# akshatvasisht/janus

Hardware: AMD Instinct MI355X
Metric: xRT (audio-s/wall-s) per GPU, 30s clips batch=64; p50 encode+decode latency (higher is better)
Workload: dtype fp16

## Files before the change

### include/janus_kernels.h

```cpp
#ifndef JANUS_KERNELS_H_
#define JANUS_KERNELS_H_

#include <stddef.h>
#include <stdint.h>
#include "janus.h"

#ifdef __cplusplus
extern "C" {
#endif

enum { JANUS_EPI_F16 = 0, JANUS_EPI_GELU_F16 = 1, JANUS_EPI_RESID_F32 = 2, JANUS_EPI_F32 = 3 };
enum { JANUS_ACT_NONE = 0, JANUS_ACT_SILU = 1, JANUS_ACT_GELU = 2, JANUS_ACT_TANH = 3 };

int janus_gemm_f16(int epi, const uint16_t* A, int64_t lda, const uint16_t* W, int64_t ldw,
                   const float* bias, void* C, int64_t ldc, const float* R, int64_t ldr, int M,
                   int N, int K, void* stream);

int janus_gemm_nt128_f16(int epi, const uint16_t* A, int64_t lda, const uint16_t* W, int64_t ldw,
                         const float* bias, void* C, int64_t ldc, const float* R, int64_t ldr, int M,
                         int N, int K, void* stream);

int janus_gemm_lt_f16(int epi, const uint16_t* A, int64_t lda, const uint16_t* W, int64_t ldw,
                      const float* bias, void* C, int64_t ldc, const float* R, int64_t ldr, int M,
                      int N, int K, void* stream);
// ... 38 lines not shown

int janus_cross_attention_f16(const uint16_t* qk, const uint16_t* enc, int batch, int Te, int D,
                              int H, int nsplit, float* part_c, float* part_ml, uint16_t* out,
                              void* stream);

int janus_decode_attention_f16(const uint16_t* q, int64_t q_bs, const uint16_t* k,
                               const uint16_t* v, int64_t kv_bs, int64_t kv_rs, int Tkv,
                               uint16_t* out, int64_t o_bs, int batch, int H, float scale,
                               float* part_o, float* part_ml, void* stream);

int janus_np_voiced_mean_f32(const float* values, const int64_t* offsets, int batch,
                             float* mean_out, int32_t* count_out, void* stream);

int janus_sample_gumbel_f32(const uint32_t* seeds, int batch, int pos, int V, float* out,
                            void* stream);

int janus_beam_partial_blocks(int V, int K, int max_blocks);
int janus_beam_logits_topk_f16(const uint16_t* A, const uint16_t* W, int K, int V, int batch,
                               int eot, int suppress_blank, int blank, int ts_begin,
                               int no_timestamps, int max_initial_ts, const uint8_t* smask,
                               const int32_t* row_rules, int max_blocks, void* parts, void* tops,
                               int n2k, float* all_v, int32_t* all_i, float* ts_v, int32_t* ts_i,
                               void* stream);
int janus_beam_step(const void* parts, const void* tops, int nblk, int eot, int suppress_blank,
                    int blank, int ts_begin, int no_timestamps, int max_initial_ts,
                    int32_t* row_rules, int32_t* tokens, int ld, int pos, int32_t* done,
                    float* sum_lp, int32_t* n_tok, const int32_t* plen, int beam_size,
                    int n_windows, int32_t* nlive, int32_t* nfin, int32_t* wdone, int32_t* moved,
                    int32_t* parent, int32_t* fin_tok, float* fin_s, int32_t* fin_n, void* stream);
int janus_beam_reorder_f16(uint16_t* kc, uint16_t* vc, int layers, int n_windows, int beam_size,
                           int n_ctx, int d, int pos, const int32_t* parent, const int32_t* moved,
                           void* stream);

int janus_decode_plan_describe(const janus_whisper_config* cfg, const janus_decode_options* opt,
                               const janus_decode_rows* rows, int batch, int cus, int resident,
                               int multi_lane, float temperature, const float* temperatures,
                               int beam_size, const int32_t* stand, int n_stand, int stand_maxlen,
                               char* text, int text_cap, int64_t* key, int key_cap, int32_t* n_key);

int janus_align_dtw_f32(const float* x, int N, int F, uint8_t* trace, int32_t* text_indices,
                        int32_t* time_indices, int32_t* path_len, void* stream);
int janus_align_reduce_f32(const float* probs, int heads, int n, int F, int sot_len, float* A,
                           void* stream);
int janus_align_token_prob_f16(const float* x, const float* gamma, const float* beta,
                               const uint16_t* W, int rows, int d, int V, const int32_t* target,
                               float* prob, void* stream);

int janus_lang_head_f16(const float* x, const float* gamma, const float* beta, const uint16_t* emb,
                        int d, int lang_begin, int n_lang, int rows, float* probs, int32_t* best,
                        void* stream);

#ifdef __cplusplus
}
#endif
#endif
```

### janus_amd/_native.py

```python
import ctypes

import numpy as np
import os

import torch

LIB_PATH = os.path.join(os.path.dirname(os.path.abspath(__file__)), "libjanus_hip.so")
if os.environ.get("JANUS_LIB"):
    LIB_PATH = os.path.join(os.path.dirname(os.path.abspath(__file__)), os.path.basename(os.environ["JANUS_LIB"]))


class JanusNativeError(RuntimeError):
    """A libjanus_hip.so entry point returned a non-zero status."""


class janus_value(ctypes.Structure):
    _fields_ = [("type", ctypes.c_int32), ("i", ctypes.c_int64), ("f", ctypes.c_double),
                ("s", ctypes.c_char_p), ("len", ctypes.c_size_t)]


class janus_packet(ctypes.Structure):
    _fields_ = [("text", ctypes.c_char_p), ("text_len", ctypes.c_size_t),
                ("mode", ctypes.c_int64), ("n_prosody", ctypes.c_int32),
                ("prosody_keys", ctypes.POINTER(janus_value)),
# ... 60 lines not shown
    "janus_vocoder_set_tensor": [_P, ctypes.c_char_p, _P, _I64],
    "janus_vocoder_frontend": [_P, _P, _P, _P, _I32, _I32, _P, _P],
    "janus_vocoder_frontend_ex": [_P, _P, _P, _P, _P, _I32, _I32, _P, _P],
    "janus_vocoder_speaker": [_P, _P, _P, _I32, _P, _P],
    "janus_vocoder_forward": [_P, _P, _I32, _I32, _P, _P, _P],
    "janus_vocoder_forward_ex": [_P, _P, _I32, _I32, _P, _P, _P, _P],
    "janus_vocoder_set_timing": [_P, _I32],
    "janus_vocoder_conv_stats": [_P, _P, _P, _P, _I32],
    "janus_vocoder_family_stats": [_P, _I32, _P, _P, _P, _P, _P, _P, _I32],
    "janus_gemm_f16": [_I32, _P, _I64, _P, _I64, _P, _P, _I64, _P, _I64, _I32, _I32, _I32, _P],
    "janus_gemm_nt128_f16": [_I32, _P, _I64, _P, _I64, _P, _P, _I64, _P, _I64, _I32, _I32, _I32, _P],
    "janus_gemm_lt_f16": [_I32, _P, _I64, _P, _I64, _P, _P, _I64, _P, _I64, _I32, _I32, _I32, _P],
    "janus_layernorm_f16": [_P, _P, _P, _P, _I32, _I32, _F32, _P],
    "janus_wave_xor_f32": [_P, _P, _I32, _P],
    "janus_quant_rows_i8": [_P, _I64, _P, _I64, _P, _I32, _I32, _P],
    "janus_layernorm_quant_i8": [_P, _P, _P, _P, _P, _I32, _I32, _F32, _P],
    "janus_gemm_i8": [_I32, _P, _I64, _P, _I64, _P, _P, _P, _P, _I64, _P, _I64, _I32, _I32, _I32, _P],
    "janus_resid_ln_f16": [_P, _I64, _P, _I64, _P, _P, _P, _P, _F32, _P, _I32, _I32, _I32, _P],
    "janus_gemm_ln_f16": [_I32, _P, _I64, _P, _P, _F32, _P, _I64, _P, _P, _I64, _I32, _I32, _I32, _P],
    "janus_attention_f16": [_P, _P, _I32, _I32, _I32, _F32, _P],
    "janus_conv1d_packed_size": [_I32, _I32, _I32, _I32, _I32],
    "janus_conv1d_pack": [_P, _P, _I32, _I32, _I32, _I32, _I32, _P],
    "janus_conv1d_f16": [_P, _I32, _I32, _I32, _P, _P, _P, _I32, _I32, _I32, _I32, _I32, _I32,
                         _I32, _I32, _I32, _P, _I64, _F32, _I32, _P],
    "janus_resunit_packed_size": [_I32, _I32],
    "janus_resunit_pack": [_P, _P, _I32, _I32, _P],
    "janus_resunit_f16": [_P, _P, _P, _P, _P, _P, _I32, _I32, _I32, _I32, _I32, _F32, _I32, _P],
    "janus_cross_attention_f16": [_P, _P, _I32, _I32, _I32, _I32, _I32, _P, _P, _P, _P],
    "janus_decode_attention_f16": [_P, _I64, _P, _P, _I64, _I64, _I32, _P, _I64, _I32, _I32, _F32,
                                   _P, _P, _P],
    "janus_beam_partial_blocks": [_I32, _I32, _I32],
    "janus_beam_logits_topk_f16": [_P, _P, _I32, _I32, _I32, _I32, _I32, _I32, _I32, _I32, _I32, _P, _P,
                                   _I32, _P, _P, _I32, _P, _P, _P, _P, _P],
    "janus_beam_step": [_P, _P, _I32, _I32, _I32, _I32, _I32, _I32, _I32, _P, _P, _I32, _I32, _P, _P, _P,
                        _P, _I32, _I32, _P, _P, _P, _P, _P, _P, _P, _P, _P],
    "janus_beam_reorder_f16": [_P, _P, _I32, _I32, _I32, _I32, _I32, _I32, _P, _P, _P],
    "janus_align_dtw_f32": [_P, _I32, _I32, _P, _P, _P, _P, _P],
    "janus_align_reduce_f32": [_P, _I32, _I32, _I32, _I32, _P, _P],
    "janus_align_token_prob_f16": [_P, _P, _P, _P, _I32, _I32, _I32, _P, _P, _P],
    "janus_whisper_detect_language": [_P, _P, _I32, _I32, _I32, _I32, _P, _P, _P],
    "janus_lang_head_f16": [_P, _P, _P, _P, _I32, _I32, _I32, _I32, _P, _P, _P],
    "janus_decode_plan_describe": [_P, _P, _P, _I32, _I32, _I32, _I32, _F32, _P, _I32, _P, _I32, _I32,
                                   _P, _I32, _P, _I32, _P],
}
RESTYPES = {"janus_conv1d_packed_size": ctypes.c_int64}

_lib = None


def lib() -> ctypes.CDLL:
    global _lib
    if _lib is None:
        if not os.path.exists(LIB_PATH):
            raise ImportError(
                f"{LIB_PATH} is missing: build it with `python -c 'import __graft_entry__ as g; "
                "g.build()'` (hipcc --offload-arch=gfx950). janus_amd has no CPU fallback.")
        l = ctypes.CDLL(LIB_PATH)
        l.janus_last_error.restype = ctypes.c_char_p
        l.janus_last_error.argtypes = []
        for name, argtypes in SIGNATURES.items():
            if os.environ.get("JANUS_LIB") and not hasattr(l, name):
                continue
            fn = getattr(l, name)
            fn.argtypes = argtypes
            fn.restype = RESTYPES.get(name, ctypes.c_int)
        _lib = l
    return _lib


def check(rc: int) -> None:
    if rc != 0:
        raise JanusNativeError(lib().janus_last_error().decode("utf-8", "replace"))


def call(name: str, *args) -> None:
    check(getattr(lib(), name)(*args))


# ... 55 lines not shown
```

### janus_amd/csrc/decode.cpp

```cpp
#include <algorithm>
#include <condition_variable>
#include <cstring>
#include <thread>
#include <type_traits>
#include "decoder.h"
#include "dec_persist.h"
#include "decode_plan.h"
#include "whisper_internal.h"

namespace janus {

struct LaneLatch {
  std::mutex m;
  std::condition_variable cv;
  int left = 0;
  void arrive(bool wait) {
    std::unique_lock<std::mutex> lk(m);
    if (--left == 0) cv.notify_all();
    if (wait) cv.wait(lk, [&] { return left <= 0; });
  }
};
struct LaneArrival {
  LaneLatch* l;
  bool done = false;
// ... 407 lines not shown
    _Float16* ck = ckeys + (int64_t)l * Me * d;
    _Float16* cv = cvals + (int64_t)l * Me * d;
    if (fused_ln) {
      gemm_skinny_ln_launch(EPI_F16, lnargs(L.ln2g, L.ln2b, L.wq_c.as<_Float16>(), L.bq_c, q2, d, d,
                                            nullptr, nullptr, pos), s);
    } else {
      if (!ln_fuse && !lnp2 && !rln2) layernorm_launch(x, L.ln2g, L.ln2b, a, B, d, 1e-5f, s);
      gemm_launch(EPI_F16, with_ln(dgargs(a, d, L.wq_c.as<_Float16>(), d, L.bq_c, q2, d, B, d, d),
                                   L.ln2g, L.ln2b, lnp2), s);
    }
    decode_attention_split_launch(q2, d, ck, cv, (int64_t)Te * d, d, Te, o, d, B, H, scale, part_o,
                                  part_ml, s);
    if (rln3) resid_ln(o, L.wo_c, L.bo_c, L.ln3g, L.ln3b);
    else resid(o, d, L.wo_c, L.bo_c, L.ln3g, L.ln3b);
  }

  void mlp(int l, int pos) const {
    DecLayer& L = w->dec[l];
    if (fused_ln) {
      gemm_skinny_ln_launch(EPI_GELU_F16, lnargs(L.ln3g, L.ln3b, L.w1.as<_Float16>(), L.b1, f, 4 * d,
                                                 4 * d, nullptr, nullptr, pos), s);
    } else {
      if (!ln_fuse && !lnp3 && !rln3) layernorm_launch(x, L.ln3g, L.ln3b, a, B, d, 1e-5f, s);
      gemm_launch(EPI_GELU_F16, with_ln(dgargs(a, d, L.w1.as<_Float16>(), d, L.b1, f, 4 * d, B, 4 * d, d),
                                        L.ln3g, L.ln3b, lnp3), s);
    }
    resid(f, 4 * d, L.w2, L.b2, l + 1 < nl ? w->dec[l + 1].ln1g : fin_g,
          l + 1 < nl ? w->dec[l + 1].ln1b : fin_b);
  }

  void tail(int pos) const {
    const int nblk = P.nblk, nwin = P.nwin;
    if (!ln_fuse && !lnp_fin && !layerk) layernorm_launch(x, fin_g, fin_b, a, B, d, 1e-5f, s);
    logits_partial_launch(a, d, w->tok16.as<_Float16>(), d, V, B, R, smask,
                          rules, parts, s,
                          lnp_fin ? x : nullptr, d, fin_g, fin_b, P.lg_cap,
                          P.sampling ? seed : nullptr, pos,
                          P.row_temps ? itemp : nullptr,
                          P.beam_k ? btop : nullptr);
    if (P.beam_k) {
      beam_step_launch(parts, btop, nblk, R, rules,
                       tokens, maxlen, pos, done, sum_lp, n_tokens, prompt,
                       nsp, bst, nwin, s);
      if (pos + 1 < maxlen - 1)
        beam_reorder_launch(kcache, vcache, nl, nwin, P.beam_k, NC, d, pos,
                            bst.parent, bst.moved, s);
      return;
    }
    if (P.fuse_se && pos + 1 < maxlen - 1)
      select_embed_launch(parts, nblk, R, rules, tokens,
                          maxlen, pos, done, sum_lp, n_tokens, B, s, prompt,
                          nsp, w->tok16.as<_Float16>(), pos_emb, d, x,
                          fused_ln ? lnp : nullptr, w->dec[0].ln1g, w->dec[0].ln1b,
                          (ln_fuse || (embed_ln && !layerk)) ? a : nullptr, roff);
    else
      select_partials_launch(parts, nblk, R, rules, tokens,
                             maxlen, pos, done, sum_lp, n_tokens, B, s, prompt,
                             nsp, roff);
  }

  void forward(int pos) const {
    if (!(P.fuse_se && pos >= P.sample_begin && pos > 0))
      embed_launch(w->tok16.as<_Float16>(), pos_emb, tokens, maxlen, pos, d, x,
                   fused_ln ? lnp : nullptr, B, s, w->dec[0].ln1g, w->dec[0].ln1b,
                   (ln_fuse || (embed_ln && !layerk)) ? a : nullptr, roff);
    for (int l = 0; l < nl; ++l) {
      DecLayer& L = w->dec[l];
// ... 429 lines not shown
```

### janus_amd/csrc/decoder.h

```cpp
#pragma once
#include "common.h"
#include "decode_shapes.h"

namespace janus {

struct RowRules {
  int sample_begin;
  int suppress_all_ts;
  int suppress_text;
  int ts_floor;
  int last_stamp;
  int pad[3];
};

struct LogitPart {
  float m_all, s_all;
  float m_text;
  float m_ts, s_ts;
  float b_all_v; int b_all_i;
  float b_ts_v; int b_ts_i;
  float t_v;
  float m_raw, s_raw;
  float b_all_r, b_ts_r;
};
// ... 4 lines not shown
  float tv[kBeamTop]; int ti[kBeamTop];
};

__host__ __device__ inline uint32_t noise_mix(uint32_t h) {
  h ^= h >> 16; h *= 0x85ebca6bu; h ^= h >> 13; h *= 0xc2b2ae35u; h ^= h >> 16;
  return h;
}
__host__ __device__ inline uint32_t noise_base(uint32_t seed, int pos) {
  return noise_mix(seed ^ noise_mix((uint32_t)pos * 0x9e3779b9u + 0x7f4a7c15u));
}
__device__ inline float sample_gumbel(uint32_t base, int token) {
  const uint32_t h = noise_mix(base ^ ((uint32_t)token * 0x27d4eb2fu));
  const float u = (float)((h >> 8) | 1u) * 0x1p-24f;
  return -logf(-logf(u));
}

void cast_f16_f32_launch(const _Float16* in, float* out, int64_t n, hipStream_t s);
void cast_f32_f16_launch(const float* in, _Float16* out, int64_t n, hipStream_t s);
void embed_launch(const _Float16* tok_emb, const float* pos_emb, const int32_t* tokens,
                  int ld_tokens, int pos, int d, float* x, float2* part, int B, hipStream_t s,
                  const float* ln_g = nullptr, const float* ln_b = nullptr,
                  _Float16* ln_out = nullptr, const int32_t* roff = nullptr);
void kv_store_launch(const _Float16* qkv, int d, int pos, int n_ctx, _Float16* kc, _Float16* vc,
                     int B, hipStream_t s);
void init_tokens_launch(int32_t* tokens, int ld, const int32_t* prompt, int plen, int32_t* done,
                        float* sum_lp, int32_t* n_tok, int B, hipStream_t s);
void init_counters_launch(int32_t* done, float* sum_lp, int32_t* n_tok, float* nsp, int B,
                          hipStream_t s);
void select_launch(const float* logits, int V, const DecodeRules& R, const uint8_t* smask,
                   int32_t* tokens, int ld, int pos, int sample_begin_pos, int32_t* done,
                   float* sum_lp, int32_t* n_tok, int B, hipStream_t s);
void rules_init_launch(RowRules* rules, int B, hipStream_t s);
int logits_partial_blocks(int V, int K, int max_blocks = 256);
void logits_partial_launch(const _Float16* A, int lda, const _Float16* W, int K, int V, int B,
                           const DecodeRules& R, const uint8_t* smask, const RowRules* rules,
                           LogitPart* parts, hipStream_t s,
                           const float* lnx = nullptr, int ldx = 0, const float* ln_g = nullptr,
                           const float* ln_b = nullptr, int max_blocks = 256,
                           const uint32_t* seeds = nullptr, int pos = 0,
                           const float* row_inv_temp = nullptr, BeamTop* tops = nullptr);
void select_partials_launch(const LogitPart* parts, int nblk, const DecodeRules& R,
                            RowRules* rules, int32_t* tokens, int ld, int pos, int32_t* done,
                            float* sum_lp, int32_t* n_tok, int B, hipStream_t s,
                            const int32_t* plen = nullptr, float* nsp = nullptr,
                            const int32_t* roff = nullptr);
void select_embed_launch(const LogitPart* parts, int nblk, const DecodeRules& R, RowRules* rules,
                         int32_t* tokens, int ld, int pos, int32_t* done, float* sum_lp,
                         int32_t* n_tok, int B, hipStream_t s, const int32_t* plen, float* nsp,
                         const _Float16* tok_emb, const float* pos_emb, int d, float* x,
                         float2* part, const float* ln_g, const float* ln_b, _Float16* ln_out,
                         const int32_t* roff = nullptr);
void build_mask_launch(const int32_t* list, int n, uint8_t* mask, int V, hipStream_t s);
void sample_gumbel_launch(const uint32_t* seeds, int B, int pos, int V, float* out, hipStream_t s);

struct BeamState {
  int k;
  float length_penalty;
  int32_t* nlive;
  int32_t* nfin;
  int32_t* wdone;
  int32_t* moved;
  int32_t* parent;
  int32_t* fin_tok;
  float* fin_s;
  int32_t* fin_n;
};
void beam_init_launch(const BeamState& st, int W, hipStream_t s);
// ... 15 lines not shown
```

### janus_amd/csrc/decoder.hip

```cpp
#include <algorithm>
#include <cfloat>
#include <cstdlib>
#ifdef JANUS_DEBUG_ASSERT
#include <cassert>
#endif
#include "mfma.h"
#include "kernels.h"
#include "decoder.h"
#include "decoder_dev.h"

namespace janus {

__global__ void cast_f16_f32_kernel(const _Float16* __restrict__ in, float* __restrict__ out,
                                    int64_t n) {
  const int64_t i = (int64_t)blockIdx.x * blockDim.x + threadIdx.x;
  if (i < n) out[i] = (float)in[i];
}

void cast_f16_f32_launch(const _Float16* in, float* out, int64_t n, hipStream_t s) {
  if (n <= 0) return;
  cast_f16_f32_kernel<<<(unsigned)cdiv(n, 256), 256, 0, s>>>(in, out, n);
  JANUS_LAUNCH_CHECK();
}

// ... 294 lines not shown
__global__ void build_mask_kernel(const int32_t* __restrict__ list, int n, uint8_t* __restrict__ mask,
                                  int V) {
  const int i = blockIdx.x * blockDim.x + threadIdx.x;
  if (i < n && list[i] >= 0 && list[i] < V) mask[list[i]] = 1;
}


__global__ void rules_init_kernel(RowRules* rules, int B) {
  const int b = blockIdx.x * blockDim.x + threadIdx.x;
  if (b >= B) return;
  RowRules r;
  r.sample_begin = 1;
  r.suppress_all_ts = r.suppress_text = 0;
  r.ts_floor = -1;
  r.last_stamp = -1;
  r.pad[0] = r.pad[1] = r.pad[2] = 0;
  rules[b] = r;
}

void rules_init_launch(RowRules* rules, int B, hipStream_t s) {
  rules_init_kernel<<<(B + 63) / 64, 64, 0, s>>>(rules, B);
  JANUS_LAUNCH_CHECK();
}

constexpr int lg_waves(int ) { return 8; }
int logits_partial_blocks(int V, int K, int max_blocks) {
  const int cap = max_blocks > 0 ? max_blocks : 256;
  return std::max(1, std::min(cap, ((V + 15) / 16 + lg_waves(K) - 1) / lg_waves(K)));
}


template <int NKS, int NB, bool SAMPLE, bool BEAM = false>
__global__ __launch_bounds__(lg_waves(NKS * 32) * 64) void logits_partial_kernel(
    const _Float16* __restrict__ A, int lda, const _Float16* __restrict__ W, int V, int B,
    DecodeRules R, const uint8_t* __restrict__ smask, const RowRules* __restrict__ rules,
    LogitPart* __restrict__ parts, int ntiles, const float* __restrict__ lnx, int ldx,
    const float* __restrict__ ln_g, const float* __restrict__ ln_b, int rot,
    const uint32_t* __restrict__ seeds, int pos, const float* __restrict__ rinv,
    BeamTop* __restrict__ tops) {
  extern __shared__ __attribute__((aligned(16))) _Float16 lg_smem[];
  dec_wave_prio();
  {
    const int r0 = (int)blockIdx.y * 64;
    A += (int64_t)r0 * lda;
    rules += r0;
    parts += (int64_t)r0 * gridDim.x;
    if (lnx) lnx += (int64_t)r0 * ldx;
    if (seeds) seeds += r0;
    if (rinv) rinv += r0;
    if (BEAM) tops += (int64_t)r0 * gridDim.x;
    B = min(64, B - r0);
  }
  constexpr int K = NKS * 32;
  constexpr int kLgWaves = lg_waves(K);
  constexpr int AP = K + 16;
  _Float16* sA = lg_smem;
  float* sT = reinterpret_cast<float*>(sA + 64 * AP);
  RowRules* sR = reinterpret_cast<RowRules*>(sT + kLgWaves * 64 * 17);
  const int tid = threadIdx.x, lane = tid & 63, w = wave_id();
  half8 bw[NB][NKS];
  uint4 sm16[NB];
  auto phys = [&](int t) { const int q = t + rot; return q >= ntiles ? q - ntiles : q; };
#define LG_LOAD(BUF, TILE)                                                                    \
  do {                                                                                        \
    const int bcol_ = min(phys(TILE) * 16 + (lane & 15), V - 1);                              \
    const _Float16* wrow_ = W + (int64_t)bcol_ * K + 8 * (lane >> 4);                         \
    _Pragma("unroll") for (int ks = 0; ks < NKS; ++ks)                                        \
      bw[BUF][ks] = *reinterpret_cast<const half8*>(wrow_ + 32 * ks);                         \
                 \
    sm16[BUF] = *reinterpret_cast<const uint4*>(smask + phys(TILE) * 16);                     \
  } while (0)
  const int tile0 = blockIdx.x * kLgWaves + w;
  const int stride = gridDim.x * kLgWaves;
#pragma unroll
  for (int u = 0; u < NB; ++u)
    if (tile0 + u * stride < ntiles) LG_LOAD(u, tile0 + u * stride);
  if (lnx) {
    ln_rows_wave<(K + 255) / 256, 64 / kLgWaves>(lnx, ldx, w, kLgWaves, B, ln_g, ln_b, sA, w, AP, K,
                                                 1e-5f, lane);
  } else {
    for (int i = tid; i < 64 * (K / 8); i += kLgWaves * 64) {
      const int r = i / (K / 8), c8 = (i % (K / 8)) * 8;
      uint4 v = make_uint4(0, 0, 0, 0);
      if (r < B) v = *reinterpret_cast<const uint4*>(A + (int64_t)r * lda + c8);
      *reinterpret_cast<uint4*>(sA + r * AP + c8) = v;
    }
  }
  if (tid < 64) {
    RowRules rr;
    if (tid < B) rr = rules[tid];
    else { rr.sample_begin = 0; rr.suppress_all_ts = rr.suppress_text = 0; rr.ts_floor = -1; rr.last_stamp = -1; }
    sR[tid] = rr;
  }
  __syncthreads();
  float* patch = sT + w * 64 * 17;
  const int lr = lane & 15, kc8 = 8 * (lane >> 4);
  RowRules rr;
  rr.sample_begin = sR[lane].sample_begin; rr.suppress_all_ts = sR[lane].suppress_all_ts;
  rr.suppress_text = sR[lane].suppress_text; rr.ts_floor = sR[lane].ts_floor;
  const float inv_t = SAMPLE && rinv ? rinv[min(lane, B - 1)] : R.inv_temp;
  float m_all = -INFINITY, s_all = 0.f, m_text = -INFINITY, m_ts = -INFINITY, s_ts = 0.f;
// ... 184 lines not shown
      if (w == 0 && lane < B) {
        float hv[kLgWaves];
        int hi[kLgWaves], hp[kLgWaves];
#pragma unroll
        for (int k = 0; k < kLgWaves; ++k) {
          hp[k] = 0;
          hv[k] = mv[(k * kBeamTop) * 64 + lane];
          hi[k] = mi[(k * kBeamTop) * 64 + lane];
        }
        for (int q = 0; q < kBeamTop; ++q) {
          float bv = hv[0];
          int bi = hi[0], bk = 0;
#pragma unroll
          for (int k = 1; k < kLgWaves; ++k)
            if (better(hv[k], hi[k], bv, bi)) { bv = hv[k]; bi = hi[k]; bk = k; }
          if (set) { dst->tv[q] = bv; dst->ti[q] = bi; }
          else { dst->av[q] = bv; dst->ai[q] = bi; }
#pragma unroll
          for (int k = 0; k < kLgWaves; ++k)
            if (k == bk) {
              hp[k] += 1;
              const bool in = hp[k] < kBeamTop;
              const int o = (k * kBeamTop + (in ? hp[k] : 0)) * 64 + lane;
              hv[k] = in ? mv[o] : -INFINITY;
              hi[k] = in ? mi[o] : 0x7fffffff;
            }
        }
      }
    }
  }
}
#undef LG_LOAD

void logits_partial_launch(const _Float16* A, int lda, const _Float16* W, int K, int V, int B,
                           const DecodeRules& R, const uint8_t* smask, const RowRules* rules,
                           LogitPart* parts, hipStream_t s, const float* lnx, int ldx,
                           const float* ln_g, const float* ln_b, int max_blocks,
                           const uint32_t* seeds, int pos, const float* row_inv_temp, BeamTop* tops) {
  JANUS_CHECK(!tops || !(R.inv_temp > 0.f), "logits: the beam partials are greedy only");
  JANUS_CHECK(K == 384 || K == 512 || K == 768, "logits: K (d_model) must be 384, 512 or 768");
  const bool sample = R.inv_temp > 0.f;
  JANUS_CHECK(!sample || seeds, "logits: sampling needs per-row seeds");
  const int ntiles = (V + 15) / 16;
  const int nw = lg_waves(K);
  const size_t lds = (size_t)64 * (K + 16) * 2 + (size_t)nw * 64 * 17 * 4 + 64 * sizeof(RowRules);
  auto kern = tops ? (K == 384 ? logits_partial_kernel<12, 1, false, true> : K == 512 ? logits_partial_kernel<16, 1, false, true>
                                                                        : logits_partial_kernel<24, 1, false, true>)
              : sample ? (K == 384 ? logits_partial_kernel<12, 1, true> : K == 512 ? logits_partial_kernel<16, 1, true>
                                                                          : logits_partial_kernel<24, 1, true>)
                       : (K == 384 ? logits_partial_kernel<12, 1, false> : K == 512 ? logits_partial_kernel<16, 1, false>
                                                                           : logits_partial_kernel<24, 1, false>);
  static bool attr[9] = {false, false, false, false, false, false, false, false, false};
  const int ai = (K == 384 ? 0 : K == 512 ? 1 : 2) + (tops ? 6 : sample ? 3 : 0);
  if (!attr[ai]) {
    JANUS_HIP(hipFuncSetAttribute((const void*)kern, hipFuncAttributeMaxDynamicSharedMemorySize,
                                  160 * 1024));
    attr[ai] = true;
  }
  const int grid = logits_partial_blocks(V, K, max_blocks);
  int rot = 0;
  {
    const int stride = grid * nw, rem = ntiles % stride;
    int s0 = ntiles;
    for (int t : {R.eot, R.no_timestamps, R.ts_begin})
      if (t >= 0 && t < V) s0 = std::min(s0, t / 16);
    const int nspec = ntiles - s0;
    if (rem > 0 && nspec > 0 && rem + nspec + (R.blank >= 0 ? 1 + R.blank / 16 : 0) <= stride)
      rot = ((s0 - rem) % ntiles + ntiles) % ntiles;
  }
  kern<<<dim3(grid, (B + 63) / 64), nw * 64, lds, s>>>(A, lda, W, V, B, R, smask, rules, parts, ntiles, lnx, ldx,
                                                      ln_g, ln_b, rot, seeds, pos,
                                                      sample ? row_inv_temp : nullptr, tops);
  JANUS_LAUNCH_CHECK();
}


__device__ __forceinline__ int select_row(
    const LogitPart* __restrict__ parts, int nblk, const DecodeRules& R, RowRules* __restrict__ rules,
    int32_t* __restrict__ tokens, int ld, int pos, int32_t* __restrict__ done,
    float* __restrict__ sum_lp, int32_t* __restrict__ n_tok, const int32_t* __restrict__ plen,
    float* __restrict__ nsp, const int32_t* __restrict__ roff = nullptr) {
  __shared__ LogitPart sh[4];
  const int b = blockIdx.x, tid = threadIdx.x;
  if (roff) {
    pos += roff[b];
    if (pos + 1 >= ld) return -1;
  }
  int32_t* row_tok = tokens + (int64_t)b * ld;
  const int pl = plen ? plen[b] : 1;
  if (pos + 1 < pl) {
    if (nsp && pos + 1 + R.target_back == pl) {
      const LogitPart q = row_parts_reduce(parts + (int64_t)b * nblk, nblk, sh);
      if (tid == 0) nsp[b] = R.target >= 0 ? __expf(q.t_v - (q.m_raw + __logf(q.s_raw))) : 0.f;
    }
    return row_tok[pos + 1];
  }
  if (done[b]) {
    if (tid == 0) row_tok[pos + 1] = R.eot;
    return R.eot;
  }
  const LogitPart q = row_parts_reduce(parts + (int64_t)b * nblk, nblk, sh);
  if (tid != 0) return -1;
  const float m_all = q.m_all, s_all = q.s_all, m_text = q.m_text, m_ts = q.m_ts, s_ts = q.s_ts;
// ... 91 lines not shown
```

### janus_amd/csrc/decoder_dev.h

```cpp
#pragma once
#include "mfma.h"
#include "decoder.h"

namespace janus {

__device__ __forceinline__ float lse_merge(float m1, float s1, float m2, float s2, float* mo) {
  const float m = fmaxf(m1, m2);
  *mo = m;
  if (m == -INFINITY) return 0.f;
  return s1 * __expf(m1 - m) + s2 * __expf(m2 - m);
}

__device__ __forceinline__ bool better(float v, int i, float bv, int bi) {
  return v > bv || (v == bv && i < bi);
}

__device__ __forceinline__ LogitPart row_parts_reduce(const LogitPart* __restrict__ pr, int nblk,
                                                      LogitPart* sh) {
  const int tid = threadIdx.x, lane = tid & 63, w = wave_id();
  float m_all = -INFINITY, s_all = 0.f, m_text = -INFINITY, m_ts = -INFINITY, s_ts = 0.f;
  float ba_v = -INFINITY, bt_v = -INFINITY;
  int ba_i = 0x7fffffff, bt_i = 0x7fffffff;
  float m_raw = -INFINITY, s_raw = 0.f, t_v = -INFINITY;
  float ba_r = -INFINITY, bt_r = -INFINITY;
  for (int i = tid; i < nblk; i += 256) {
    const LogitPart p = pr[i];
    float mo;
    s_all = lse_merge(m_all, s_all, p.m_all, p.s_all, &mo); m_all = mo;
    s_ts = lse_merge(m_ts, s_ts, p.m_ts, p.s_ts, &mo); m_ts = mo;
    s_raw = lse_merge(m_raw, s_raw, p.m_raw, p.s_raw, &mo); m_raw = mo;
    m_text = fmaxf(m_text, p.m_text);
    t_v = fmaxf(t_v, p.t_v);
    if (better(p.b_all_v, p.b_all_i, ba_v, ba_i)) { ba_v = p.b_all_v; ba_i = p.b_all_i; ba_r = p.b_all_r; }
    if (better(p.b_ts_v, p.b_ts_i, bt_v, bt_i)) { bt_v = p.b_ts_v; bt_i = p.b_ts_i; bt_r = p.b_ts_r; }
  }
  auto level = [&](auto shf, auto shi) __attribute__((always_inline)) {
    float mo;
    const float om = shf(m_all), os = shf(s_all);
    s_all = lse_merge(m_all, s_all, om, os, &mo); m_all = mo;
    const float tm = shf(m_ts), ts = shf(s_ts);
    s_ts = lse_merge(m_ts, s_ts, tm, ts, &mo); m_ts = mo;
    const float rm = shf(m_raw), rs = shf(s_raw);
    s_raw = lse_merge(m_raw, s_raw, rm, rs, &mo); m_raw = mo;
// ... 53 lines not shown
```

### janus_amd/csrc/kapi.cpp

```cpp
#include <algorithm>
#include <cstring>
#include <vector>
#include "align.h"
#include "devmem.h"
#include "kernels.h"
#include "decoder.h"
#include "dec_persist.h"
#include "decode_plan.h"
#include "../../include/janus_kernels.h"

namespace janus {

ConvArgs conv_args_torch(const _Float16* in, int B, int T_in, int Cin, const _Float16* packed,
                         const float* bias, _Float16* out, int T_out, int Cout, int taps,
                         int stride, int padding, int dilation, int transposed, int pre_act,
                         int post_act, const _Float16* res, int64_t res_bs, float scale,
                         int accumulate) {
  ConvArgs a{};
  a.in = in; a.in_bs = (int64_t)T_in * Cin; a.T_in = T_in; a.Cin = Cin;
  a.w = packed; a.bias = bias;
  a.out = out; a.out_bs = (int64_t)T_out * Cout; a.T_out = T_out; a.Cout = Cout;
  a.res = res; a.res_bs = res_bs;
  a.pre_act = pre_act; a.post_act = post_act; a.out_scale = scale; a.accumulate = accumulate;
  a.B = B;
  if (!transposed) {
    a.taps = taps; a.dil = dilation; a.in_stride = stride; a.in_off = -padding;
    a.out_stride = 1; a.out_off = 0; a.n_rows = T_out; a.phases = 1;
  } else {
    const int u = stride;
    a.taps = 2; a.dil = -1; a.in_stride = 1; a.in_off = 0;
    a.out_stride = u; a.out_off = -padding; a.phases = u;
    a.n_rows = (T_out + padding) / u + 1;
  }
  return a;
// ... 185 lines not shown
}

extern "C" int janus_decode_attention_f16(const uint16_t* q, int64_t q_bs, const uint16_t* k,
                                          const uint16_t* v, int64_t kv_bs, int64_t kv_rs,
                                          int Tkv, uint16_t* out, int64_t o_bs, int batch, int H,
                                          float scale, float* part_o, float* part_ml,
                                          void* stream) {
  return guarded([&] {
    JANUS_CHECK(Tkv <= 512 || (part_o && part_ml), "decode attention: scratch needed past 512 keys");
    decode_attention_split_launch(reinterpret_cast<const _Float16*>(q), q_bs,
                                  reinterpret_cast<const _Float16*>(k),
                                  reinterpret_cast<const _Float16*>(v), kv_bs, kv_rs, Tkv,
                                  reinterpret_cast<_Float16*>(out), o_bs, batch, H, scale, part_o,
                                  part_ml, (hipStream_t)stream);
  });
}

extern "C" int janus_sample_gumbel_f32(const uint32_t* seeds, int batch, int pos, int V, float* out,
                                       void* stream) {
  return guarded([&] {
    JANUS_CHECK(seeds && out, "null argument");
    sample_gumbel_launch(seeds, batch, pos, V, out, (hipStream_t)stream);
  });
}

static DecodeRules beam_rules(int eot, int suppress_blank, int blank, int ts_begin, int no_timestamps,
                              int max_initial_ts) {
  DecodeRules R;
  R.eot = eot; R.suppress_blank = suppress_blank; R.blank = blank; R.ts_begin = ts_begin;
  R.no_timestamps = no_timestamps; R.max_initial_ts = max_initial_ts; R.target = -1; R.inv_temp = 0.f;
  return R;
}

extern "C" int janus_beam_partial_blocks(int V, int K, int max_blocks) {
  return logits_partial_blocks(V, K, max_blocks);
}

extern "C" int janus_beam_logits_topk_f16(const uint16_t* A, const uint16_t* W, int K, int V, int batch,
                                          int eot, int suppress_blank, int blank, int ts_begin,
                                          int no_timestamps, int max_initial_ts, const uint8_t* smask,
                                          const int32_t* row_rules, int max_blocks, void* parts,
                                          void* tops, int n2k, float* all_v, int32_t* all_i, float* ts_v,
                                          int32_t* ts_i, void* stream) {
  return guarded([&] {
    JANUS_CHECK(A && W && smask && row_rules && parts && tops && all_v && all_i && ts_v && ts_i, "null argument");
    JANUS_CHECK(batch >= 1 && batch <= kSkinnyMaxRows, "beam_logits_topk: 1 <= batch <= 512");
    static_assert(sizeof(RowRules) == 32 && sizeof(LogitPart) == 56 && sizeof(BeamTop) == 256, "ABI sizes");
    const DecodeRules R = beam_rules(eot, suppress_blank, blank, ts_begin, no_timestamps, max_initial_ts);
    const int nblk = logits_partial_blocks(V, K, max_blocks);
    logits_partial_launch(reinterpret_cast<const _Float16*>(A), K, reinterpret_cast<const _Float16*>(W), K, V,
                          batch, R, smask, reinterpret_cast<const RowRules*>(row_rules),
                          static_cast<LogitPart*>(parts), (hipStream_t)stream, nullptr, 0, nullptr, nullptr,
                          max_blocks, nullptr, 0, nullptr, static_cast<BeamTop*>(tops));
    beam_rowtop_launch(static_cast<const BeamTop*>(tops), nblk, batch, n2k, all_v, all_i, ts_v, ts_i,
                       (hipStream_t)stream);
  });
}

extern "C" int janus_beam_step(const void* parts, const void* tops, int nblk, int eot, int suppress_blank,
                               int blank, int ts_begin, int no_timestamps, int max_initial_ts,
                               int32_t* row_rules, int32_t* tokens, int ld, int pos, int32_t* done,
                               float* sum_lp, int32_t* n_tok, const int32_t* plen, int beam_size,
                               int n_windows, int32_t* nlive, int32_t* nfin, int32_t* wdone,
                               int32_t* moved, int32_t* parent, int32_t* fin_tok, float* fin_s,
                               int32_t* fin_n, void* stream) {
  return guarded([&] {
    JANUS_CHECK(parts && tops && row_rules && tokens && done && sum_lp && n_tok && plen && nlive && nfin &&
                    wdone && moved && parent && fin_tok && fin_s && fin_n, "null argument");
    JANUS_CHECK(n_windows >= 1, "beam_step: n_windows must be >= 1");
    const DecodeRules R = beam_rules(eot, suppress_blank, blank, ts_begin, no_timestamps, max_initial_ts);
    BeamState st{};
    st.k = beam_size; st.length_penalty = 1.0f;
    st.nlive = nlive; st.nfin = nfin; st.wdone = wdone; st.moved = moved; st.parent = parent;
    st.fin_tok = fin_tok; st.fin_s = fin_s; st.fin_n = fin_n;
    beam_step_launch(static_cast<const LogitPart*>(parts), static_cast<const BeamTop*>(tops), nblk, R,
                     reinterpret_cast<RowRules*>(row_rules), tokens, ld, pos, done, sum_lp, n_tok, plen,
                     nullptr, st, n_windows, (hipStream_t)stream);
  });
}

extern "C" int janus_beam_reorder_f16(uint16_t* kc, uint16_t* vc, int layers, int n_windows, int beam_size,
                                      int n_ctx, int d, int pos, const int32_t* parent,
                                      const int32_t* moved, void* stream) {
  return guarded([&] {
    JANUS_CHECK(kc && vc && parent && moved, "null argument");
    beam_reorder_launch(reinterpret_cast<_Float16*>(kc), reinterpret_cast<_Float16*>(vc), layers, n_windows,
                        beam_size, n_ctx, d, pos, parent, moved, (hipStream_t)stream);
  });
// ... 110 lines not shown
```

### janus_amd/csrc/whisper.cpp

```cpp
#include <algorithm>
#include <cstdlib>
#include <cstring>
#include "decoder.h"
#include "whisper_internal.h"

namespace janus {

static _Float16* to_f16(const float* src, int64_t n, DevMem& dst, hipStream_t s) {
  dst.ensure(sizeof(_Float16) * n);
  cast_f32_f16_launch(src, dst.as<_Float16>(), n, s);
  return dst.as<_Float16>();
}

static void fuse_f16(const ParamStore& P, const std::vector<std::string>& names, int64_t each,
                     DevMem& dst, hipStream_t s) {
  dst.ensure(sizeof(_Float16) * each * names.size());
  for (size_t i = 0; i < names.size(); ++i) {
    _Float16* d = dst.as<_Float16>() + i * each;
    if (P.has(names[i])) cast_f32_f16_launch(P.get(names[i], each), d, each, s);
    else JANUS_HIP(hipMemsetAsync(d, 0, sizeof(_Float16) * each, s));
  }
}

static void fuse_f32(const ParamStore& P, const std::vector<std::string>& names, int64_t each,
                     DevMem& dst, hipStream_t s) {
  dst.ensure(sizeof(float) * each * names.size());
  for (size_t i = 0; i < names.size(); ++i) {
    float* d = dst.as<float>() + i * each;
    if (P.has(names[i]))
      JANUS_HIP(hipMemcpyAsync(d, P.get(names[i], each), sizeof(float) * each,
                               hipMemcpyDeviceToDevice, s));
    else JANUS_HIP(hipMemsetAsync(d, 0, sizeof(float) * each, s));
  }
}

void prepare(janus_whisper* w, hipStream_t s) {
  if (w->prepared) return;
  JANUS_HIP(hipDeviceSynchronize());
  for (auto& lane : w->lanes) lane->drop_graphs();
  const auto& c = w->cfg;
  const int d = c.d_model, ff = 4 * d;
  const ParamStore& P = w->params;
  auto pk = [&](const std::string& name, int cin, DevMem& dst) {
    const float* src = P.get(name, (int64_t)d * cin * 3);
    const ConvPack g = conv_pack_geometry(cin, d, 3);
    dst.ensure(sizeof(_Float16) * g.phase_elems);
    conv_pack_weights(src, dst.as<_Float16>(), cin, d, 3, 0, 1, s);
  };
  pk("encoder.conv1.weight", c.n_mels, w->conv1p);
  pk("encoder.conv2.weight", d, w->conv2p);
  to_f16(P.get("encoder.embed_positions.weight", (int64_t)c.n_audio_ctx * d),
         (int64_t)c.n_audio_ctx * d, w->pos16, s);
  to_f16(P.get("decoder.embed_tokens.weight", (int64_t)c.n_vocab * d), (int64_t)c.n_vocab * d,
         w->tok16, s);
  const int64_t dd = (int64_t)d * d, fd = (int64_t)ff * d;
  w->enc.clear();
  w->enc.resize(c.enc_layers);
  w->i8_prepared = false;
  for (int l = 0; l < c.enc_layers; ++l) {
    const std::string p = "encoder.layers." + std::to_string(l) + ".";
    EncLayer& L = w->enc[l];
    fuse_f16(P, {p + "self_attn.q_proj.weight", p + "self_attn.k_proj.weight", p + "self_attn.v_proj.weight"}, dd, L.wqkv, s);
    fuse_f32(P, {p + "self_attn.q_proj.bias", p + "self_attn.k_proj.bias", p + "self_attn.v_proj.bias"}, d, L.bqkv, s);
    to_f16(P.get(p + "self_attn.out_proj.weight", dd), dd, L.wo, s);
    to_f16(P.get(p + "fc1.weight", fd), fd, L.w1, s);
    to_f16(P.get(p + "fc2.weight", fd), fd, L.w2, s);
    L.bo = P.get(p + "self_attn.out_proj.bias", d);
    L.b1 = P.get(p + "fc1.bias", ff);
    L.b2 = P.get(p + "fc2.bias", d);
    L.ln1g = P.get(p + "self_attn_layer_norm.weight", d);
    L.ln1b = P.get(p + "self_attn_layer_norm.bias", d);
    L.ln2g = P.get(p + "final_layer_norm.weight", d);
    L.ln2b = P.get(p + "final_layer_norm.bias", d);
  }
  w->dec.clear();
  w->dec.resize(c.dec_layers);
  for (int l = 0; l < c.dec_layers; ++l) {
    const std::string p = "decoder.layers." + std::to_string(l) + ".";
    DecLayer& L = w->dec[l];
    fuse_f16(P, {p + "self_attn.q_proj.weight", p + "self_attn.k_proj.weight", p + "self_attn.v_proj.weight"}, dd, L.wqkv, s);
    fuse_f32(P, {p + "self_attn.q_proj.bias", p + "self_attn.k_proj.bias", p + "self_attn.v_proj.bias"}, d, L.bqkv, s);
    to_f16(P.get(p + "self_attn.out_proj.weight", dd), dd, L.wo, s);
    to_f16(P.get(p + "encoder_attn.q_proj.weight", dd), dd, L.wq_c, s);
    to_f16(P.get(p + "encoder_attn.k_proj.weight", dd), dd, L.wk_c, s);
    to_f16(P.get(p + "encoder_attn.v_proj.weight", dd), dd, L.wv_c, s);
    to_f16(P.get(p + "encoder_attn.out_proj.weight", dd), dd, L.wo_c, s);
    to_f16(P.get(p + "fc1.weight", fd), fd, L.w1, s);
// ... 242 lines not shown
```

### janus_amd/csrc/whisper_internal.h

```cpp
#pragma once
#include <map>
#include <memory>
#include <mutex>
#include <vector>
#include "align.h"
#include "devmem.h"
#include "kernels.h"
#include "../../include/janus.h"

namespace janus {

struct EncLayer {
  DevMem wqkv, bqkv, wo, w1, w2;
  DevMem qqkv, sqkv, qo, so, q1, s1, q2, s2;
  const float *bo, *b1, *b2, *ln1g, *ln1b, *ln2g, *ln2b;
};
struct DecLayer {
  DevMem wqkv, bqkv, wo, wq_c, wk_c, wv_c, wo_c, w1, w2;
  DevMem wqk, bqk;
  const float *bo, *bq_c, *bv_c, *bo_c, *b1, *b2;
  const float *ln1g, *ln1b, *ln2g, *ln2b, *ln3g, *ln3b;
};

struct DecLane {
// ... 11 lines not shown
  hipStream_t stream = nullptr;
  std::vector<uint32_t> stream_mask;
  hipEvent_t ev_done = nullptr;
  uint32_t* h_segerr = nullptr;
  hipEvent_t ev_segerr = nullptr;
  bool segerr_pending = false;
  DecLane() = default;
  DecLane(const DecLane&) = delete;
  DecLane& operator=(const DecLane&) = delete;
  void drop_graphs() {
    for (auto& kv : graphs) (void)hipGraphExecDestroy(kv.second);
    graphs.clear();
    graph_nodes.clear();
  }
  ~DecLane() {
    drop_graphs();
    if (stream) (void)hipStreamDestroy(stream);
    if (ev_done) (void)hipEventDestroy(ev_done);
    if (ev_segerr) (void)hipEventDestroy(ev_segerr);
    if (h_segerr) (void)hipHostFree(h_segerr);
  }
};

}

struct janus_whisper {
  janus_whisper_config cfg;
  janus::ParamStore params;
  bool prepared = false;
  int enc_compute = JANUS_ENC_COMPUTE_F16;
  bool i8_prepared = false;
  std::mutex mu;
  janus::DevMem conv1p, conv2p, pos16, tok16;
  std::vector<janus::EncLayer> enc;
  std::vector<janus::DecLayer> dec;
  janus::DevMem ws_x1, ws_x2, ws_r, ws_a, ws_qkv, ws_o, ws_f, ws_logmel, ws_maxkey;
  janus::DevMem ws_q8, ws_qs;
  std::vector<std::unique_ptr<janus::DecLane>> lanes;
  int last_slot = 0;
  std::unique_ptr<janus::DecLane> lang_lane;
  janus::AlignState align;
  hipEvent_t ev_in = nullptr;
  ~janus_whisper() {
    if (ev_in) (void)hipEventDestroy(ev_in);
  }
};

namespace janus {

void prepare(janus_whisper* w, hipStream_t s);

inline GemmArgs gargs(const _Float16* A, int64_t lda, const _Float16* W, int64_t ldw,
                      const float* bias, void* C, int64_t ldc, int M, int N, int K,
                      const float* R = nullptr, int64_t ldr = 0) {
  GemmArgs g;
  g.A = A; g.lda = lda; g.W = W; g.ldw = ldw; g.bias = bias; g.C = C; g.ldc = ldc;
  g.R = R; g.ldr = ldr; g.M = M; g.N = N; g.K = K;
  return g;
}

}
```

Before: 6173.

## Pack vocab embedding into tile-contiguous layout and load via buffer descriptors

Adds a one-time repack of the token embedding into 16-row by 32-column tiles, so that each wave's 128-bit loads in the logits kernel become fully contiguous. The loads are issued through raw buffer loads with a wave-uniform base taken via readfirstlane. The aim is better coalescing and fewer address computations in the memory-bound vocab projection during decoding. The cost is extra device memory for a second copy of the embedding. A new API also repacks on the fly per call when given an unpacked matrix, and the LSE merge now uses an fma.

```diff
diff --git a/include/janus_kernels.h b/include/janus_kernels.h
--- a/include/janus_kernels.h
+++ b/include/janus_kernels.h
@@ -94,6 +94,16 @@
                            int n_ctx, int d, int pos, const int32_t* parent, const int32_t* moved,
                            void* stream);
 
+int64_t janus_vocab_pack_index(int row, int k, int K);
+int64_t janus_vocab_pack_elems(int V, int K);
+int janus_vocab_pack_f16(const uint16_t* W, int V, int K, uint16_t* packed, void* stream);
+int janus_logits_partials_f16(const uint16_t* A, const uint16_t* W, int w_packed, int K, int V,
+                              int batch, int eot, int suppress_blank, int blank, int ts_begin,
+                              int no_timestamps, int max_initial_ts, int target,
+                              const uint8_t* smask, const int32_t* row_rules, int max_blocks,
+                              const uint32_t* seeds, int pos, float inv_temp,
+                              const float* row_inv_temp, void* parts, void* stream);
+
 int janus_decode_plan_describe(const janus_whisper_config* cfg, const janus_decode_options* opt,
                                const janus_decode_rows* rows, int batch, int cus, int resident,
                                int multi_lane, float temperature, const float* temperatures,
diff --git a/janus_amd/_native.py b/janus_amd/_native.py
--- a/janus_amd/_native.py
+++ b/janus_amd/_native.py
@@ -116,6 +116,11 @@
     "janus_beam_partial_blocks": [_I32, _I32, _I32],
     "janus_beam_logits_topk_f16": [_P, _P, _I32, _I32, _I32, _I32, _I32, _I32, _I32, _I32, _I32, _P, _P,
                                    _I32, _P, _P, _I32, _P, _P, _P, _P, _P],
+    "janus_vocab_pack_index": [_I32, _I32, _I32],
+    "janus_vocab_pack_elems": [_I32, _I32],
+    "janus_vocab_pack_f16": [_P, _I32, _I32, _P, _P],
+    "janus_logits_partials_f16": [_P, _P, _I32, _I32, _I32, _I32, _I32, _I32, _I32, _I32, _I32, _I32, _I32,
+                                  _P, _P, _I32, _P, _I32, _F32, _P, _P, _P],
     "janus_beam_step": [_P, _P, _I32, _I32, _I32, _I32, _I32, _I32, _I32, _P, _P, _I32, _I32, _P, _P, _P,
                         _P, _I32, _I32, _P, _P, _P, _P, _P, _P, _P, _P, _P],
     "janus_beam_reorder_f16": [_P, _P, _I32, _I32, _I32, _I32, _I32, _I32, _P, _P, _P],
@@ -127,7 +132,8 @@
     "janus_decode_plan_describe": [_P, _P, _P, _I32, _I32, _I32, _I32, _F32, _P, _I32, _P, _I32, _I32,
                                    _P, _I32, _P, _I32, _P],
 }
-RESTYPES = {"janus_conv1d_packed_size": ctypes.c_int64}
+RESTYPES = {"janus_conv1d_packed_size": ctypes.c_int64, "janus_vocab_pack_index": ctypes.c_int64,
+            "janus_vocab_pack_elems": ctypes.c_int64}
 
 _lib = None
 
diff --git a/janus_amd/csrc/decode.cpp b/janus_amd/csrc/decode.cpp
--- a/janus_amd/csrc/decode.cpp
+++ b/janus_amd/csrc/decode.cpp
@@ -463,7 +463,7 @@
   void tail(int pos) const {
     const int nblk = P.nblk, nwin = P.nwin;
     if (!ln_fuse && !lnp_fin && !layerk) layernorm_launch(x, fin_g, fin_b, a, B, d, 1e-5f, s);
-    logits_partial_launch(a, d, w->tok16.as<_Float16>(), d, V, B, R, smask,
+    logits_partial_launch(a, d, w->tokpk.as<_Float16>(), d, V, B, R, smask,
                           rules, parts, s,
                           lnp_fin ? x : nullptr, d, fin_g, fin_b, P.lg_cap,
                           P.sampling ? seed : nullptr, pos,
diff --git a/janus_amd/csrc/decoder.h b/janus_amd/csrc/decoder.h
--- a/janus_amd/csrc/decoder.h
+++ b/janus_amd/csrc/decoder.h
@@ -60,7 +60,13 @@
                    float* sum_lp, int32_t* n_tok, int B, hipStream_t s);
 void rules_init_launch(RowRules* rules, int B, hipStream_t s);
 int logits_partial_blocks(int V, int K, int max_blocks = 256);
-void logits_partial_launch(const _Float16* A, int lda, const _Float16* W, int K, int V, int B,
+__host__ __device__ inline int64_t vocab_pack_index(int row, int k, int K) {
+  const int t = row >> 4, ks = k >> 5, l = (row & 15) + 16 * ((k & 31) >> 3);
+  return (((int64_t)t * (K >> 5) + ks) * 64 + l) * 8 + (k & 7);
+}
+inline int64_t vocab_pack_elems(int V, int K) { return (int64_t)((V + 15) / 16) * 16 * K; }
+void vocab_pack_launch(const _Float16* W, int V, int K, _Float16* packed, hipStream_t s);
+void logits_partial_launch(const _Float16* A, int lda, const _Float16* Wp, int K, int V, int B,
                            const DecodeRules& R, const uint8_t* smask, const RowRules* rules,
                            LogitPart* parts, hipStream_t s,
                            const float* lnx = nullptr, int ldx = 0, const float* ln_g = nullptr,
diff --git a/janus_amd/csrc/decoder.hip b/janus_amd/csrc/decoder.hip
--- a/janus_amd/csrc/decoder.hip
+++ b/janus_amd/csrc/decoder.hip
@@ -350,7 +350,7 @@
 
 template <int NKS, int NB, bool SAMPLE, bool BEAM = false>
 __global__ __launch_bounds__(lg_waves(NKS * 32) * 64) void logits_partial_kernel(
-    const _Float16* __restrict__ A, int lda, const _Float16* __restrict__ W, int V, int B,
+    const _Float16* __restrict__ A, int lda, const _Float16* __restrict__ Wp, int V, int B,
     DecodeRules R, const uint8_t* __restrict__ smask, const RowRules* __restrict__ rules,
     LogitPart* __restrict__ parts, int ntiles, const float* __restrict__ lnx, int ldx,
     const float* __restrict__ ln_g, const float* __restrict__ ln_b, int rot,
@@ -381,10 +381,12 @@
   auto phys = [&](int t) { const int q = t + rot; return q >= ntiles ? q - ntiles : q; };
 #define LG_LOAD(BUF, TILE)                                                                    \
   do {                                                                                        \
-    const int bcol_ = min(phys(TILE) * 16 + (lane & 15), V - 1);                              \
-    const _Float16* wrow_ = W + (int64_t)bcol_ * K + 8 * (lane >> 4);                         \
+    const int pt_ = __builtin_amdgcn_readfirstlane(phys(TILE));                               \
+    const __amdgpu_buffer_rsrc_t rs_ = __builtin_amdgcn_make_buffer_rsrc(                     \
+        const_cast<_Float16*>(Wp + (int64_t)pt_ * (16 * K)), 0, 32 * K, 0x00020000);          \
     _Pragma("unroll") for (int ks = 0; ks < NKS; ++ks)                                        \
-      bw[BUF][ks] = *reinterpret_cast<const half8*>(wrow_ + 32 * ks);                         \
+      bw[BUF][ks] = __builtin_bit_cast(                                                       \
+          half8, __builtin_amdgcn_raw_buffer_load_b128(rs_, lane * 16, ks * 1024, 0));        \
                  \
     sm16[BUF] = *reinterpret_cast<const uint4*>(smask + phys(TILE) * 16);                     \
   } while (0)
@@ -635,7 +637,26 @@
 }
 #undef LG_LOAD
 
-void logits_partial_launch(const _Float16* A, int lda, const _Float16* W, int K, int V, int B,
+__global__ void vocab_pack_kernel(const _Float16* __restrict__ W, int V, int K,
+                                  _Float16* __restrict__ packed, int64_t n16) {
+  const int64_t i = (int64_t)blockIdx.x * blockDim.x + threadIdx.x;
+  if (i >= n16) return;
+  const int l = (int)(i & 63), nks = K >> 5;
+  const int ks = (int)((i >> 6) % nks), t = (int)((i >> 6) / nks);
+  const int row = 16 * t + (l & 15), k = 32 * ks + 8 * (l >> 4);
+  uint4 v = make_uint4(0, 0, 0, 0);
+  if (row < V) v = *reinterpret_cast<const uint4*>(W + (int64_t)row * K + k);
+  *reinterpret_cast<uint4*>(packed + vocab_pack_index(row, k, K)) = v;
+}
+
+void vocab_pack_launch(const _Float16* W, int V, int K, _Float16* packed, hipStream_t s) {
+  JANUS_CHECK(V >= 1 && K >= 32 && K % 32 == 0, "vocab_pack: K must be a multiple of 32");
+  const int64_t n16 = vocab_pack_elems(V, K) / 8;
+  vocab_pack_kernel<<<(unsigned)((n16 + 255) / 256), 256, 0, s>>>(W, V, K, packed, n16);
+  JANUS_LAUNCH_CHECK();
+}
+
+void logits_partial_launch(const _Float16* A, int lda, const _Float16* Wp, int K, int V, int B,
                            const DecodeRules& R, const uint8_t* smask, const RowRules* rules,
                            LogitPart* parts, hipStream_t s, const float* lnx, int ldx,
                            const float* ln_g, const float* ln_b, int max_blocks,
@@ -671,7 +692,7 @@
     if (rem > 0 && nspec > 0 && rem + nspec + (R.blank >= 0 ? 1 + R.blank / 16 : 0) <= stride)
       rot = ((s0 - rem) % ntiles + ntiles) % ntiles;
   }
-  kern<<<dim3(grid, (B + 63) / 64), nw * 64, lds, s>>>(A, lda, W, V, B, R, smask, rules, parts, ntiles, lnx, ldx,
+  kern<<<dim3(grid, (B + 63) / 64), nw * 64, lds, s>>>(A, lda, Wp, V, B, R, smask, rules, parts, ntiles, lnx, ldx,
                                                       ln_g, ln_b, rot, seeds, pos,
                                                       sample ? row_inv_temp : nullptr, tops);
   JANUS_LAUNCH_CHECK();
diff --git a/janus_amd/csrc/decoder_dev.h b/janus_amd/csrc/decoder_dev.h
--- a/janus_amd/csrc/decoder_dev.h
+++ b/janus_amd/csrc/decoder_dev.h
@@ -8,7 +8,7 @@
   const float m = fmaxf(m1, m2);
   *mo = m;
   if (m == -INFINITY) return 0.f;
-  return s1 * __expf(m1 - m) + s2 * __expf(m2 - m);
+  return fmaf(s1, __expf(m1 - m), s2 * __expf(m2 - m));
 }
 
 __device__ __forceinline__ bool better(float v, int i, float bv, int bi) {
diff --git a/janus_amd/csrc/kapi.cpp b/janus_amd/csrc/kapi.cpp
--- a/janus_amd/csrc/kapi.cpp
+++ b/janus_amd/csrc/kapi.cpp
@@ -1,5 +1,6 @@
 #include <algorithm>
 #include <cstring>
+#include <memory>
 #include <vector>
 #include "align.h"
 #include "devmem.h"
@@ -251,6 +252,17 @@
   return R;
 }
 
+struct PackedVocab {
+  DevMem mem;
+  hipStream_t s;
+  PackedVocab(const _Float16* W, int V, int K, hipStream_t stream) : s(stream) {
+    mem.ensure(sizeof(_Float16) * vocab_pack_elems(V, K));
+    vocab_pack_launch(W, V, K, mem.as<_Float16>(), s);
+  }
+  ~PackedVocab() { (void)hipStreamSynchronize(s); }
+  const _Float16* get() const { return mem.as<_Float16>(); }
+};
+
 extern "C" int janus_beam_partial_blocks(int V, int K, int max_blocks) {
   return logits_partial_blocks(V, K, max_blocks);
 }
@@ -267,12 +279,49 @@
     static_assert(sizeof(RowRules) == 32 && sizeof(LogitPart) == 56 && sizeof(BeamTop) == 256, "ABI sizes");
     const DecodeRules R = beam_rules(eot, suppress_blank, blank, ts_begin, no_timestamps, max_initial_ts);
     const int nblk = logits_partial_blocks(V, K, max_blocks);
-    logits_partial_launch(reinterpret_cast<const _Float16*>(A), K, reinterpret_cast<const _Float16*>(W), K, V,
+    const PackedVocab wp(reinterpret_cast<const _Float16*>(W), V, K, (hipStream_t)stream);
+    logits_partial_launch(reinterpret_cast<const _Float16*>(A), K, wp.get(), K, V,
                           batch, R, smask, reinterpret_cast<const RowRules*>(row_rules),
                           static_cast<LogitPart*>(parts), (hipStream_t)stream, nullptr, 0, nullptr, nullptr,
                           max_blocks, nullptr, 0, nullptr, static_cast<BeamTop*>(tops));
     beam_rowtop_launch(static_cast<const BeamTop*>(tops), nblk, batch, n2k, all_v, all_i, ts_v, ts_i,
                        (hipStream_t)stream);
+  });
+}
+
+extern "C" int64_t janus_vocab_pack_index(int row, int k, int K) { return vocab_pack_index(row, k, K); }
+
+extern "C" int64_t janus_vocab_pack_elems(int V, int K) { return vocab_pack_elems(V, K); }
+
+extern "C" int janus_vocab_pack_f16(const uint16_t* W, int V, int K, uint16_t* packed, void* stream) {
+  return guarded([&] {
+    JANUS_CHECK(W && packed, "null argument");
+    vocab_pack_launch(reinterpret_cast<const _Float16*>(W), V, K, reinterpret_cast<_Float16*>(packed),
+                      (hipStream_t)stream);
+  });
+}
+
+extern "C" int janus_logits_partials_f16(const uint16_t* A, const uint16_t* W, int w_packed, int K, int V,
+                                         int batch, int eot, int suppress_blank, int blank, int ts_begin,
+                                         int no_timestamps, int max_initial_ts, int target,
+                                         const uint8_t* smask, const int32_t* row_rules, int max_blocks,
+                                         const uint32_t* seeds, int pos, float inv_temp,
+                                         const float* row_inv_temp, void* parts, void* stream) {
+  return guarded([&] {
+    JANUS_CHECK(A && W && smask && row_rules && parts, "null argument");
+    JANUS_CHECK(batch >= 1 && batch <= kSkinnyMaxRows, "logits_partials: 1 <= batch <= 512");
+    static_assert(sizeof(RowRules) == 32 && sizeof(LogitPart) == 56, "ABI sizes");
+    DecodeRules R = beam_rules(eot, suppress_blank, blank, ts_begin, no_timestamps, max_initial_ts);
+    R.target = target;
+    R.inv_temp = !seeds ? 0.f : row_inv_temp ? 1.0f : inv_temp;
+    JANUS_CHECK(!seeds || R.inv_temp > 0.f, "logits_partials: sampling needs inv_temp > 0 or per-row values");
+    std::unique_ptr<PackedVocab> tmp;
+    if (!w_packed) tmp.reset(new PackedVocab(reinterpret_cast<const _Float16*>(W), V, K, (hipStream_t)stream));
+    logits_partial_launch(reinterpret_cast<const _Float16*>(A), K,
+                          tmp ? tmp->get() : reinterpret_cast<const _Float16*>(W), K, V, batch, R, smask,
+                          reinterpret_cast<const RowRules*>(row_rules), static_cast<LogitPart*>(parts),
+                          (hipStream_t)stream, nullptr, 0, nullptr, nullptr, max_blocks, seeds, pos,
+                          row_inv_temp, nullptr);
   });
 }
 
diff --git a/janus_amd/csrc/whisper.cpp b/janus_amd/csrc/whisper.cpp
--- a/janus_amd/csrc/whisper.cpp
+++ b/janus_amd/csrc/whisper.cpp
@@ -53,6 +53,8 @@
          (int64_t)c.n_audio_ctx * d, w->pos16, s);
   to_f16(P.get("decoder.embed_tokens.weight", (int64_t)c.n_vocab * d), (int64_t)c.n_vocab * d,
          w->tok16, s);
+  w->tokpk.ensure(sizeof(_Float16) * vocab_pack_elems(c.n_vocab, d));
+  vocab_pack_launch(w->tok16.as<_Float16>(), c.n_vocab, d, w->tokpk.as<_Float16>(), s);
   const int64_t dd = (int64_t)d * d, fd = (int64_t)ff * d;
   w->enc.clear();
   w->enc.resize(c.enc_layers);
diff --git a/janus_amd/csrc/whisper_internal.h b/janus_amd/csrc/whisper_internal.h
--- a/janus_amd/csrc/whisper_internal.h
+++ b/janus_amd/csrc/whisper_internal.h
@@ -67,6 +67,7 @@
   bool i8_prepared = false;
   std::mutex mu;
   janus::DevMem conv1p, conv2p, pos16, tok16;
+  janus::DevMem tokpk;
   std::vector<janus::EncLayer> enc;
   std::vector<janus::DecLayer> dec;
   janus::DevMem ws_x1, ws_x2, ws_r, ws_a, ws_qkv, ws_o, ws_f, ws_logmel, ws_maxkey;
```

New measurement: 6230, median of 4. Within noise of the previous version (+0.9%).
